# eikehmueller/mlmcpathintegral

Hardware: AMD Instinct MI355X
Metric: lattice-site-updates/sec (higher is better)
Workload: dtype f64

## Files before the change

mlmcpathintegral_amd/csrc/schwinger_perm.hpp:

```cpp
#pragma once
#include "lattice_sweep.hpp"

namespace mlmcpi {

#ifdef MLMCPI_STAMPS
__device__ unsigned long long g_stamps[16 * 65536];
#define MLMCPI_STAMP(k)                                                                                            \
  do {                                                                                                             \
    if (threadIdx.x == 0 && blockIdx.y * gridDim.x + blockIdx.x < 65536)                                           \
      g_stamps[(blockIdx.y * gridDim.x + blockIdx.x) * 16 + (k)] = __builtin_amdgcn_s_memrealtime();               \
  } while (0)
#define MLMCPI_STAMP_WHERE()                                                                                       \
  do {                                                                                                             \
    if (threadIdx.x == 0 && blockIdx.y * gridDim.x + blockIdx.x < 65536)                                           \
      g_stamps[(blockIdx.y * gridDim.x + blockIdx.x) * 16 + 15] =                                                  \
          ((unsigned long long)__builtin_amdgcn_s_getreg((20 ) | (0 << 6) | (31 << 11)) << 32) |         \
          __builtin_amdgcn_s_getreg((4 ) | (0 << 6) | (31 << 11));                                        \
  } while (0)
#else
#define MLMCPI_STAMP(k) do { } while (0)
#define MLMCPI_STAMP_WHERE() do { } while (0)
#endif

#ifndef MLMCPI_PERM_U
#define MLMCPI_PERM_U 0
#endif

template <class PG>
struct PermPlane {
  static constexpr int kRow = PG::kPitch * 8, kStep = kRow + 8;
  static constexpr uint32_t QB = (uint32_t)PG::kQRows * kRow;
  static_assert(kStep == (int)PG::kStep * 8, "the stride of a stream");
  uint32_t K;
  __device__ __forceinline__ explicit PermPlane(uint32_t K_) : K(K_) {}
  __device__ __forceinline__ bool has_col(uint32_t C) const { return (C & 1u) ? C <= PG::col_last(K, 1) : C >= PG::col_first(K, 0) && C <= PG::col_last(K, 0); }
  __device__ __forceinline__ bool has_row(uint32_t R) const { return (R & 1u) ? R <= PG::row_last(K, 1) : R >= PG::row_first(K, 0) && R <= PG::row_last(K, 0); }
  __device__ __forceinline__ uint32_t col(uint32_t C) const { return (C & 1u) ? QB + PG::col_u(K, C) * 8u : PG::col_u(K, C) * 8u; }
  __device__ __forceinline__ uint32_t row(uint32_t R) const { return (R & 1u) ? 2u * QB + PG::row_v(K, R) * (uint32_t)kRow : PG::row_v(K, R) * (uint32_t)kRow; }
};

struct PermBuildPos {
  uint32_t c, r, rend, row_off, gj;
  uint32_t cb;
  const double2 *src;
  uint32_t col;
  bool active, owns;
};
template <int NT, class PP>
__device__ __forceinline__ PermBuildPos perm_build_pos(const PP &P, const double2 *__restrict__ src, uint32_t Mt, uint32_t Mx, uint32_t gi0,
                                                       uint32_t gj0, uint32_t W, uint32_t rows) {
  PermBuildPos q;
  const uint32_t wave = __builtin_amdgcn_readfirstlane(threadIdx.x / kWave), lane = threadIdx.x % kWave;
  const uint32_t nwc = W > 63 ? 2 : 1;
  const uint32_t groups = (NT / kWave) >> (nwc - 1);
  const uint32_t g = wave >> (nwc - 1), cw = wave & (nwc - 1);
  static_assert(((NT / kWave) & (NT / kWave - 1)) == 0, "waves per workgroup: a power of two (shifts for divisions)");
  const uint32_t rpg = groups == 4 ? (rows + 3) >> 2 : groups == 8 ? (rows + 7) >> 3 : (rows + groups - 1) / groups;
  q.c = 63 * cw + lane;
  q.r = __builtin_amdgcn_readfirstlane(g * rpg);
  q.rend = __builtin_amdgcn_readfirstlane(g < groups ? min(rows, q.r + rpg) : 0);
  q.active = q.r < q.rend;
  q.owns = lane < 63 && q.c < W && P.has_col(q.c);
  q.cb = P.col(q.c);
  q.src = src;
  q.col = wrap_add(gi0, min(q.c, W), Mt);
  q.gj = __builtin_amdgcn_readfirstlane(wrap_add(gj0, q.r, Mx));
  q.row_off = q.gj * Mt;
  return q;
}
template <int U>
__device__ __forceinline__ void perm_rows_load(PermBuildPos &q, uint32_t Mt, uint32_t Mx, bool first, double2 &cur, double2 (&nxt)[U]) {
  if (!q.active) return;
  if (first) cur = (q.src + q.row_off)[q.col];
#pragma unroll
  for (int u = 0; u < U; ++u) {
    q.gj = q.gj + 1 == Mx ? 0 : q.gj + 1;
    q.row_off = q.gj == 0 ? 0 : q.row_off + Mt;
    if (q.r + u < q.rend) nxt[u] = (q.src + q.row_off)[q.col];
  }
}
template <int U, class PP>
__device__ __forceinline__ void perm_rows_store(PermBuildPos &q, const PP &P, double *plane, double2 &cur, const double2 (&nxt)[U]) {
  if (!q.active) return;
  char *const pb = reinterpret_cast<char *>(plane) + q.cb;
#pragma unroll
  for (int u = 0; u < U; ++u)
    if (q.r + u < q.rend) {
      const double right = wave_rotate_down(cur.y);
      if (q.owns && P.has_row(q.r + u)) *reinterpret_cast<double *>(pb + P.row(q.r + u)) = ((cur.x + right) - nxt[u].x) - cur.y;
      cur = nxt[u];
    }
  q.r += U;
}
template <int NT, int U, bool ONCE, class PP>
__device__ __forceinline__ void perm_build_rows(const PP &P, double *plane, const double2 *__restrict__ src, uint32_t Mt, uint32_t Mx,
                                                uint32_t gi0, uint32_t gj0, uint32_t W, uint32_t rows) {
  PermBuildPos q = perm_build_pos<NT>(P, src, Mt, Mx, gi0, gj0, W, rows);
  double2 cur = make_double2(0., 0.);
  if (ONCE) {
    double2 nxt[U];
    perm_rows_load<U>(q, Mt, Mx, true, cur, nxt);
    perm_rows_store<U>(q, P, plane, cur, nxt);
    return;
  }
  bool first = true;
  while (__builtin_amdgcn_readfirstlane(q.r) < __builtin_amdgcn_readfirstlane(q.rend)) {
    double2 nxt[U];
    perm_rows_load<U>(q, Mt, Mx, first, cur, nxt);
    perm_rows_store<U>(q, P, plane, cur, nxt);
    first = false;
  }
}

template <int NT, int RING, int TH = 64>
struct PermTasks {
  using PG = PermGeom<NT, RING, TH>;
  static constexpr int OW = PG::OW, HR = PG::HR, H2 = HR / 2, NW = NT / kWave, NS = (HR + NW - 1) / NW;
  static constexpr int XC = OW - 64;
  static constexpr int L0 = XC * H2, L1 = (XC / 2) * HR;
  static constexpr int NL0 = (L0 + 63) / 64, NL1 = (L1 + 63) / 64;
  static constexpr int WF = HR - NW * (NS - 1);
  static_assert(PG::NV == NS, "slots per thread");
  static_assert(NL0 + NL1 <= NW - WF, "the left-over wave-tasks fit the free last slots");
  uint32_t wave, lane, c_mu0, c_mu1, r_lo;
  __device__ PermTasks() {
    wave = __builtin_amdgcn_readfirstlane(threadIdx.x / kWave);
    lane = threadIdx.x % kWave;
    c_mu0 = lane < 32 ? 2 * lane : 2 * (lane - 32) + 1;
    c_mu1 = 2 * (lane & 31u);
    r_lo = lane >> 5;
  }
  __device__ __forceinline__ bool task(int k, bool &mu1, uint32_t &r, uint32_t &c) const {
    const uint32_t m = wave + (uint32_t)(NW * k);
    mu1 = false; r = 0; c = 0;
    if (NW * k + NW - 1 < H2 || m < (uint32_t)H2) {
      r = 2 * m;
      c = c_mu0;
      return true;
    }
    if (m < (uint32_t)HR) {
      mu1 = true;
      r = 2 * (m - H2) + r_lo;
      c = c_mu1;
      return true;
    }
    if (XC > 0 && k == NS - 1) {
      const uint32_t j = wave - (uint32_t)WF;
      if (j < (uint32_t)NL0) {
        const uint32_t L = 64 * j + lane;
        r = 2 * (L / (XC ? XC : 1));
        c = 64 + L % (XC ? XC : 1);
        return L < (uint32_t)L0;
      }
      if (j < (uint32_t)(NL0 + NL1)) {
        const uint32_t L = 64 * (j - NL0) + lane;
        mu1 = true;
        r = L / (XC > 1 ? XC / 2 : 1);
        c = 64 + 2 * (L % (XC > 1 ? XC / 2 : 1));
        return L < (uint32_t)L1;
      }
    }
    return false;
  }
  __device__ __forceinline__ bool valid(int k) const {
    bool mu1; uint32_t r, c;
    return task(k, mu1, r, c);
  }
  __device__ __forceinline__ bool is_mu1(int k) const {
    bool mu1; uint32_t r, c;
    task(k, mu1, r, c);
    return mu1;
  }
  __device__ __forceinline__ void coords(int k, uint32_t &r, uint32_t &c) const {
    bool mu1;
    task(k, mu1, r, c);
  }
};

template <int STEP>
__device__ __forceinline__ void perm_gather5(uint32_t pa, uint32_t px, uint32_t px2, double &S, double &X, double &X2) {
  double a0 = lds_read_f64<0>(pa), x0 = lds_read_f64<0>(px), y0 = lds_read_f64<0>(px2);
  double a1 = lds_read_f64<STEP>(pa), x1 = lds_read_f64<STEP>(px), y1 = lds_read_f64<STEP>(px2);
  double a2 = lds_read_f64<2 * STEP>(pa), x2 = lds_read_f64<2 * STEP>(px), y2 = lds_read_f64<2 * STEP>(px2);
  double a3 = lds_read_f64<3 * STEP>(pa), x3 = lds_read_f64<3 * STEP>(px), y3 = lds_read_f64<3 * STEP>(px2);
  double a4 = lds_read_f64<4 * STEP>(pa), x4 = lds_read_f64<4 * STEP>(px), y4 = lds_read_f64<4 * STEP>(px2);
  asm volatile("s_waitcnt lgkmcnt(0)"
               : "+v"(a0), "+v"(x0), "+v"(y0), "+v"(a1), "+v"(x1), "+v"(y1), "+v"(a2), "+v"(x2), "+v"(y2), "+v"(a3), "+v"(x3), "+v"(y3),
                 "+v"(a4), "+v"(x4), "+v"(y4)
               :
               : "memory");
  S += a0; X += x0; X2 += y0;
  S += a1; X += x1; X2 += y1;
  S += a2; X += x2; X2 += y2;
  S += a3; X += x3; X2 += y3;
  S += a4; X += x4; X2 += y4;
}
__device__ __forceinline__ void perm_gather1(uint32_t pa, uint32_t px, uint32_t px2, double &S, double &X, double &X2) {
  double a0 = lds_read_f64<0>(pa), x0 = lds_read_f64<0>(px), y0 = lds_read_f64<0>(px2);
  asm volatile("s_waitcnt lgkmcnt(0)" : "+v"(a0), "+v"(x0), "+v"(y0) : : "memory");
  S += a0; X += x0; X2 += y0;
}

template <int NT, int RING, int TH = 64>
__device__ __forceinline__ void perm_sweeps(double *plane, const double2 *__restrict__ src, uint32_t Mt, uint32_t Mx, uint32_t i0,
                                            uint32_t j0, uint32_t K, double2 (&res)[2][PermGeom<NT, RING, TH>::NV]) {
  using PG = PermGeom<NT, RING, TH>;
  using PP = PermPlane<PG>;
  constexpr int HR = PG::HR, NV = PG::NV;
  constexpr int kGroups = NT / kWave / 2;
  constexpr int U = MLMCPI_PERM_U ? MLMCPI_PERM_U : (2 * HR + 4 * (int)kPermMaxK + kGroups - 1) / kGroups;
  const uint32_t W = PG::width(K), rows = PG::rows(K), H = RING + 2 * K;
  const PP P(K);
  auto back = [](uint32_t x, uint32_t h, uint32_t n) { return h <= n ? (x >= h ? x - h : x + n - h) : (x + n - h % n) % n; };
  const uint32_t gi0 = back(i0, H, Mt), gj0 = back(j0, H, Mx);
  const uint32_t oi0 = back(i0, RING, Mt), oj0 = back(j0, RING, Mx);
  const PermTasks<NT, RING, TH> tasks;
  const char *const src_b = reinterpret_cast<const char *>(src);
  const bool small_lattice = Mx < (uint32_t)(2 * HR + 2) || Mt < (uint32_t)(PG::OW + 2);
  auto load_theta_of = [&](int h, double2 (&th)[NV], auto small) {
#pragma unroll
    for (int k = 0; k < NV; ++k) {
      if (!tasks.valid(k)) continue;
      uint32_t r, c;
      tasks.coords(k, r, c);
      uint32_t gr = oj0 + r + h * HR, gc = oi0 + c;
      gr = min(gr, gr - Mx);
      gc = min(gc, gc - Mt);
      if ((bool)small) {
        gr = min(gr, gr - Mx); gr = min(gr, gr - Mx);
        gc = min(gc, gc - Mt); gc = min(gc, gc - Mt);
      }
      const uint32_t o = (gr * Mt + gc) * 16u;
      if (!tasks.is_mu1(k)) {
        const uint32_t o2 = gr + 1 == Mx ? o - gr * Mt * 16u : o + Mt * 16u;
        th[k] = make_double2(*reinterpret_cast<const double *>(src_b + o), *reinterpret_cast<const double *>(src_b + o2));
      } else {
        const uint32_t o2 = gc + 1 == Mt ? o - gc * 16u : o + 16u;
        th[k] = make_double2(*reinterpret_cast<const double *>(src_b + o + 8u), *reinterpret_cast<const double *>(src_b + o2 + 8u));
      }
    }
  };
  auto load_theta = [&](int h, double2 (&th)[NV]) {
    if (small_lattice) load_theta_of(h, th, std::true_type{}); else load_theta_of(h, th, std::false_type{});
  };
  auto gather = [&](int h, double2 (&d)[NV]) {
    const uint32_t lds0 = (uint32_t)(uintptr_t)plane;
#pragma unroll
    for (int k = 0; k < NV; ++k) {
      if (!tasks.valid(k)) continue;
      uint32_t r, c;
      tasks.coords(k, r, c);
      const uint32_t ro = r + (uint32_t)(h * HR), cq = c >> 1, rq = ro >> 1;
      uint32_t a, x, x2;
      if (!tasks.is_mu1(k)) {
        const uint32_t cb = (c & 1u) ? PP::QB + ((uint32_t)(PG::OW / 2 - 1) - cq) * 8u : cq * 8u;
        x = cb + rq * (uint32_t)PP::kRow;
        x2 = x + (uint32_t)PP::kRow;
        a = cb + 2u * PP::QB + ((uint32_t)(HR - 1) - rq) * (uint32_t)PP::kRow;
      } else {
        const uint32_t rb = (ro & 1u) ? 2u * PP::QB + ((uint32_t)(HR - 1) - rq) * (uint32_t)PP::kRow : (rq + 1u) * (uint32_t)PP::kRow;
        x = rb + cq * 8u;
        x2 = x + 8u;
        a = rb + PP::QB + ((uint32_t)(PG::OW / 2) - cq) * 8u;
      }
      uint32_t pa = lds0 + a, px = lds0 + x, px2 = lds0 + x2;
      double S = 0.0, X = 0.0, X2 = 0.0;
      uint32_t s = 0;
      for (; s + 5 <= K; s += 5) {
        perm_gather5<PP::kStep>(pa, px, px2, S, X, X2);
        pa += 5 * PP::kStep;
        px += 5 * PP::kStep;
        px2 += 5 * PP::kStep;
      }
      for (; s < K; ++s) {
        perm_gather1(pa, px, px2, S, X, X2);
        pa += PP::kStep;
        px += PP::kStep;
        px2 += PP::kStep;
      }
      d[k] = tasks.is_mu1(k) ? make_double2(X - S, X2 - S) : make_double2(S - X, S - X2);
    }
  };
  auto finish = [&](const double2 (&th)[NV], double2 (&d)[NV]) {
#pragma unroll
    for (int k = 0; k < NV; ++k)
      if (tasks.valid(k)) d[k] = make_double2(mod_2pi_fast(th[k].x + d[k].x), mod_2pi_fast(th[k].y + d[k].y));
  };

  perm_build_rows<NT, U, MLMCPI_PERM_U == 0>(P, plane, src, Mt, Mx, gi0, gj0, W, rows);
  double2 th[NV];
  load_theta(0, th);
  __syncthreads();
  MLMCPI_STAMP(1);
  gather(0, res[0]);
  finish(th, res[0]);
  MLMCPI_STAMP(2);
  load_theta(1, th);
  gather(1, res[1]);
  finish(th, res[1]);
}

template <int NT, int RING, int TH = 64>
__device__ __forceinline__ void perm_store_image(double *th0, double *th1, const double2 (&res)[2][PermGeom<NT, RING, TH>::NV]) {
  using PG = PermGeom<NT, RING, TH>;
  constexpr int OW = PG::OW, HR = PG::HR, NV = PG::NV;
  const PermTasks<NT, RING, TH> tasks;
#pragma unroll
  for (int h = 0; h < 2; ++h)
#pragma unroll
    for (int k = 0; k < NV; ++k) {
      if (!tasks.valid(k)) continue;
      uint32_t r, c;
      tasks.coords(k, r, c);
      const uint32_t o = (r + h * HR) * OW + c;
      if (!tasks.is_mu1(k)) {
        th0[o] = res[h][k].x;
        th0[o + OW] = res[h][k].y;
      } else {
        th1[o] = res[h][k].x;
        th1[o + 1] = res[h][k].y;
      }
    }
}

}
```

Before: 1093 billion.

## Pair mu0/mu1 tasks per wave and load both link components as double2

Reassigns the per-wave task slots so that each even/odd slot pair covers the mu0 and mu1 rows of the same row pair. Theta can then be fetched as full double2 loads with a wave-uniform row, instead of separate scattered scalar loads per component. The mu1 values are redistributed across lanes with permlane32_swap. The mod-2pi finish step is also fused into the gather loop per slot, with asm pins on the results. This adds cross-lane exchange instructions and new task-layout constraints (static asserts on NS parity) in exchange for fewer global load instructions and better coalescing.

Measured after the change: 1096 billion (median of 6 runs). No clear change (+0.3%).

```diff
diff --git a/mlmcpathintegral_amd/csrc/schwinger_perm.hpp b/mlmcpathintegral_amd/csrc/schwinger_perm.hpp
--- a/mlmcpathintegral_amd/csrc/schwinger_perm.hpp
+++ b/mlmcpathintegral_amd/csrc/schwinger_perm.hpp
@@ -116,11 +116,14 @@
 struct PermTasks {
   using PG = PermGeom<NT, RING, TH>;
   static constexpr int OW = PG::OW, HR = PG::HR, H2 = HR / 2, NW = NT / kWave, NS = (HR + NW - 1) / NW;
+  static constexpr int NP = NS / 2;
+  static constexpr int REST = H2 - NW * NP;
   static constexpr int XC = OW - 64;
   static constexpr int L0 = XC * H2, L1 = (XC / 2) * HR;
   static constexpr int NL0 = (L0 + 63) / 64, NL1 = (L1 + 63) / 64;
-  static constexpr int WF = HR - NW * (NS - 1);
+  static constexpr int WF = 2 * REST;
   static_assert(PG::NV == NS, "slots per thread");
+  static_assert(REST >= 0 && (NS % 2 == 1 || (REST == 0 && XC == 0)), "what the paired rounds leave has a last slot of its own");
   static_assert(NL0 + NL1 <= NW - WF, "the left-over wave-tasks fit the free last slots");
   uint32_t wave, lane, c_mu0, c_mu1, r_lo;
   __device__ PermTasks() {
@@ -130,21 +133,28 @@
     c_mu1 = 2 * (lane & 31u);
     r_lo = lane >> 5;
   }
+  static __device__ __forceinline__ constexpr bool paired(int k) { return k < 2 * NP; }
+  __device__ __forceinline__ uint32_t paired_row(int k) const { return 2 * (wave + (uint32_t)(NW * (k >> 1))); }
   __device__ __forceinline__ bool task(int k, bool &mu1, uint32_t &r, uint32_t &c) const {
-    const uint32_t m = wave + (uint32_t)(NW * k);
     mu1 = false; r = 0; c = 0;
-    if (NW * k + NW - 1 < H2 || m < (uint32_t)H2) {
-      r = 2 * m;
+    if (paired(k)) {
+      mu1 = (k & 1) != 0;
+      r = paired_row(k) + (mu1 ? r_lo : 0u);
+      c = mu1 ? c_mu1 : c_mu0;
+      return true;
+    }
+    if (wave < (uint32_t)REST) {
+      r = 2 * ((uint32_t)(NW * NP) + wave);
       c = c_mu0;
       return true;
     }
-    if (m < (uint32_t)HR) {
+    if (wave < (uint32_t)(2 * REST)) {
       mu1 = true;
-      r = 2 * (m - H2) + r_lo;
+      r = 2 * ((uint32_t)(NW * NP) + wave - (uint32_t)REST) + r_lo;
       c = c_mu1;
       return true;
     }
-    if (XC > 0 && k == NS - 1) {
+    if (XC > 0) {
       const uint32_t j = wave - (uint32_t)WF;
       if (j < (uint32_t)NL0) {
         const uint32_t L = 64 * j + lane;
@@ -201,6 +211,13 @@
   S += a0; X += x0; X2 += y0;
 }
 
+__device__ __forceinline__ void perm_half_exchange(double &x, double &y) {
+  const auto lo = __builtin_amdgcn_permlane32_swap((uint32_t)__double2loint(x), (uint32_t)__double2loint(y), false, false);
+  const auto hi = __builtin_amdgcn_permlane32_swap((uint32_t)__double2hiint(x), (uint32_t)__double2hiint(y), false, false);
+  x = __hiloint2double((int)hi[0], (int)lo[0]);
+  y = __hiloint2double((int)hi[1], (int)lo[1]);
+}
+
 template <int NT, int RING, int TH = 64>
 __device__ __forceinline__ void perm_sweeps(double *plane, const double2 *__restrict__ src, uint32_t Mt, uint32_t Mx, uint32_t i0,
                                             uint32_t j0, uint32_t K, double2 (&res)[2][PermGeom<NT, RING, TH>::NV]) {
@@ -218,8 +235,22 @@
   const char *const src_b = reinterpret_cast<const char *>(src);
   const bool small_lattice = Mx < (uint32_t)(2 * HR + 2) || Mt < (uint32_t)(PG::OW + 2);
   auto load_theta_of = [&](int h, double2 (&th)[NV], auto small) {
+    uint32_t gcp = oi0 + tasks.c_mu0;
+    gcp = min(gcp, gcp - Mt);
+    if ((bool)small) { gcp = min(gcp, gcp - Mt); gcp = min(gcp, gcp - Mt); }
+    const uint32_t gcb = gcp * 16u;
 #pragma unroll
     for (int k = 0; k < NV; ++k) {
+      if (tasks.paired(k)) {
+        if (k & 1) continue;
+        uint32_t gr = __builtin_amdgcn_readfirstlane(oj0 + tasks.paired_row(k) + (uint32_t)(h * HR));
+        gr = min(gr, gr - Mx);
+        if ((bool)small) { gr = min(gr, gr - Mx); gr = min(gr, gr - Mx); }
+        const uint32_t gr1 = gr + 1 == Mx ? 0 : gr + 1;
+        th[k] = *reinterpret_cast<const double2 *>(reinterpret_cast<const char *>(src + gr * Mt) + gcb);
+        th[k + 1] = *reinterpret_cast<const double2 *>(reinterpret_cast<const char *>(src + gr1 * Mt) + gcb);
+        continue;
+      }
       if (!tasks.valid(k)) continue;
       uint32_t r, c;
       tasks.coords(k, r, c);
@@ -243,11 +274,26 @@
   auto load_theta = [&](int h, double2 (&th)[NV]) {
     if (small_lattice) load_theta_of(h, th, std::true_type{}); else load_theta_of(h, th, std::false_type{});
   };
-  auto gather = [&](int h, double2 (&d)[NV]) {
+  auto pin = [](double2 &v) { asm volatile("" : "+v"(v.x), "+v"(v.y)); };
+  auto finish = [&](int k, const double2 (&th)[NV], double2 (&d)[NV]) {
+    if (tasks.paired(k)) {
+      if (!(k & 1)) return;
+      double t1x = th[k - 1].y, t1y = th[k].y;
+      perm_half_exchange(t1x, t1y);
+      d[k - 1] = make_double2(mod_2pi_fast(th[k - 1].x + d[k - 1].x), mod_2pi_fast(th[k].x + d[k - 1].y));
+      d[k] = make_double2(mod_2pi_fast(t1x + d[k].x), mod_2pi_fast(t1y + d[k].y));
+      pin(d[k - 1]);
+      pin(d[k]);
+      return;
+    }
+    d[k] = make_double2(mod_2pi_fast(th[k].x + d[k].x), mod_2pi_fast(th[k].y + d[k].y));
+    pin(d[k]);
+  };
+  auto gather = [&](int h, const double2 (&th)[NV], double2 (&d)[NV]) {
     const uint32_t lds0 = (uint32_t)(uintptr_t)plane;
 #pragma unroll
     for (int k = 0; k < NV; ++k) {
-      if (!tasks.valid(k)) continue;
+      if (!tasks.paired(k) && !tasks.valid(k)) continue;
       uint32_t r, c;
       tasks.coords(k, r, c);
       const uint32_t ro = r + (uint32_t)(h * HR), cq = c >> 1, rq = ro >> 1;
@@ -279,25 +325,18 @@
         px2 += PP::kStep;
       }
       d[k] = tasks.is_mu1(k) ? make_double2(X - S, X2 - S) : make_double2(S - X, S - X2);
+      finish(k, th, d);
     }
   };
-  auto finish = [&](const double2 (&th)[NV], double2 (&d)[NV]) {
-#pragma unroll
-    for (int k = 0; k < NV; ++k)
-      if (tasks.valid(k)) d[k] = make_double2(mod_2pi_fast(th[k].x + d[k].x), mod_2pi_fast(th[k].y + d[k].y));
-  };
-
   perm_build_rows<NT, U, MLMCPI_PERM_U == 0>(P, plane, src, Mt, Mx, gi0, gj0, W, rows);
   double2 th[NV];
   load_theta(0, th);
   __syncthreads();
   MLMCPI_STAMP(1);
-  gather(0, res[0]);
-  finish(th, res[0]);
+  gather(0, th, res[0]);
   MLMCPI_STAMP(2);
   load_theta(1, th);
-  gather(1, res[1]);
-  finish(th, res[1]);
+  gather(1, th, res[1]);
 }
 
 template <int NT, int RING, int TH = 64>
```
